# hyeeiin/ECG-Multimodal-Model

Hardware: AMD Instinct MI355X
Metric: samples/sec fwd+bwd, batch-256 multimodal (img+sig+clin), 1->8 MI355X (higher is better)
Workload: dtype bf16; 1 GPU; full multimodal (image 3x224x224 + 5000-pt signal + 16-dim clinical), fwd+bwd+Adam, encoders unfrozen; image_hw=224x224, per_gpu_batch=256, global_batch=256, parallelism=dp1

## Files before the change

ecg-multimodal-model_amd/csrc/elementwise.hip:

```cpp
#include "ops.h"

namespace {

constexpr int EW_THREADS = 256;

__device__ __forceinline__ u32x4 ld16(const void* p) { return *reinterpret_cast<const u32x4*>(p); }
__device__ __forceinline__ u32x4 ld16s(const void* p) {
#ifndef EW_NO_NT
  return __builtin_nontemporal_load(reinterpret_cast<const u32x4*>(p));
#else
  return *reinterpret_cast<const u32x4*>(p);
#endif
}
struct RowDiv { unsigned mul, sh; };
__device__ __forceinline__ long row_div(long r, RowDiv d) { return (long)(((unsigned long long)(unsigned)r * d.mul) >> d.sh); }
static RowDiv make_row_div(int d) {
  unsigned dd = d < 1 ? 1u : (unsigned)d;
  int l = 0;
  while ((1u << l) < dd) ++l;
  RowDiv r;
  r.mul = (unsigned)(((1ull << (31 + l)) + dd - 1) / dd);
  r.sh = 31u + (unsigned)l;
  return r;
}
// ... 362 lines not shown
    }
  }
}

struct BnBwdParams {
  const void* dout;
  const void* maskref;
  const float* gate;
  const float* addc;
  const void* y;
  const float* coef;
  const float* bcoef;
  void* dy;
  void* dz_out;
  float* partial;
  long M;
  int C, rows_per_sample;
  BnBwdFin fin;
  RowDiv rdiv;
  const unsigned char* mask_bits;
};

constexpr int BWD_THREADS = 1024;
template <typename T, bool APPLY>
__global__ __launch_bounds__(BWD_THREADS) void bn_bwd_kernel(BnBwdParams p) {
  constexpr int VEC = Elem<T>::VEC;
  extern __shared__ float shm_dyn[];
  float(*shm)[2 * VEC + 1] = reinterpret_cast<float(*)[2 * VEC + 1]>(shm_dyn);
  const ChanSlice cs = chan_slice(p.C);
  const int cpr = cs.W / VEC, rpi = BWD_THREADS / cpr;
  const int chunk = threadIdx.x % cpr, r0 = threadIdx.x / cpr;
  const int c0 = cs.c_lo + chunk * VEC;
  __shared__ double s_red[APPLY ? FIN_LDS_DOUBLES : 1];
  __shared__ float s_bcoef[APPLY ? 3 * 512 : 1];
  const float* bc = p.bcoef + c0;
  int bcs = p.C;
  const long rfirst = (long)blockIdx.x * rpi + r0;
  u32x4 pd = {}, pv = {};
  bool pre = APPLY && p.fin.partial != nullptr && rfirst < p.M;
  if (pre) {
    pd = ld16s((const T*)p.dout + rfirst * p.C + c0);
    pv = ld16s((const T*)p.y + rfirst * p.C + c0);
  }
  if (APPLY && p.fin.partial) {
    bn_bwd_fin_prologue<BWD_THREADS>(p.fin, p.coef, p.C, cs, s_bcoef, s_red);
    bc = s_bcoef + chunk * VEC;
    bcs = cs.W;
  }
  float mean[VEC], inv[VEC], k1[VEC], k2[VEC], k3[VEC], a1[VEC], a2[VEC], msc[VEC], msh[VEC];
#pragma unroll
  for (int j = 0; j < VEC; ++j) {
    msc[j] = p.coef[c0 + j];
    msh[j] = p.coef[p.C + c0 + j];
    mean[j] = p.coef[2 * p.C + c0 + j];
    inv[j] = p.coef[3 * p.C + c0 + j];
    a1[j] = a2[j] = 0.f;
    if (APPLY) {
      k1[j] = bc[j];
      k2[j] = bc[bcs + j];
      k3[j] = bc[2 * bcs + j];
    }
  }
  const T* dout = (const T*)p.dout;
  const T* mref = (const T*)p.maskref;
  const T* y = (const T*)p.y;
  for (long r = rfirst; r < p.M; r += (long)gridDim.x * rpi) {
    float d[VEC], m[VEC], v[VEC];
    if (pre) {
      unpack16<T>(pd, d);
      unpack16<T>(pv, v);
      pre = false;
    } else {
      unpack16<T>(ld16s(dout + r * p.C + c0), d);
      unpack16<T>(ld16s(y + r * p.C + c0), v);
    }
    if (mref == y) {
#pragma unroll
      for (int j = 0; j < VEC; ++j) d[j] = (v[j] * msc[j] + msh[j]) > 0.f ? d[j] : 0.f;
    } else if (VEC == 8 && p.mask_bits) {
      const unsigned bits = p.mask_bits[r * (p.C / VEC) + c0 / VEC];
#pragma unroll
      for (int j = 0; j < VEC; ++j) d[j] = (bits >> j) & 1u ? d[j] : 0.f;
    } else if (mref) {
      unpack16<T>(ld16s(mref + r * p.C + c0), m);
#pragma unroll
      for (int j = 0; j < VEC; ++j) d[j] = m[j] > 0.f ? d[j] : 0.f;
    }
    if (p.dz_out) st16((T*)p.dz_out + r * p.C + c0, pack16<T>(d));
    if (p.gate) {
      const float* gp = p.gate + row_div(r, p.rdiv) * p.C + c0;
#pragma unroll
      for (int j = 0; j < VEC; ++j) d[j] *= gp[j];
    }
    if (p.addc) {
      const float* ap = p.addc + row_div(r, p.rdiv) * p.C + c0;
#pragma unroll
      for (int j = 0; j < VEC; ++j) d[j] += ap[j];
    }
    if (!APPLY) {
#pragma unroll
      for (int j = 0; j < VEC; ++j) {
        float xh = (v[j] - mean[j]) * inv[j];
        a1[j] += d[j];
        a2[j] += d[j] * xh;
      }
    } else {
      float o[VEC];
#pragma unroll
      for (int j = 0; j < VEC; ++j) {
        float xh = (v[j] - mean[j]) * inv[j];
        o[j] = k1[j] * (d[j] - k2[j] - xh * k3[j]);
      }
      u32x4 pk = pack16<T>(o);
      st16((T*)p.dy + r * p.C + c0, pk);
      if (p.partial) {
        float back[VEC];
        unpack16<T>(pk, back);
#pragma unroll
        for (int j = 0; j < VEC; ++j) a1[j] += back[j];
      }
    }
  }
  if (!APPLY || p.partial) {
    constexpr int NQ = APPLY ? 1 : 2;
#pragma unroll
    for (int j = 0; j < VEC; ++j) {
      shm[threadIdx.x][j] = a1[j];
      if (!APPLY) shm[threadIdx.x][VEC + j] = a2[j];
    }
    __syncthreads();
    for (int o = threadIdx.x; o < NQ * p.C; o += BWD_THREADS) {
      int which = o / p.C, c = o % p.C;
      int ck = c / VEC, j = c % VEC;
      float s = 0.f;
      for (int k = 0; k < rpi; ++k) s += shm[k * cpr + ck][which * VEC + j];
      p.partial[(size_t)blockIdx.x * NQ * p.C + o] = s;
    }
  }
}

__global__ __launch_bounds__(1024) void bn_bwd_finalize_kernel(const float* __restrict__ partial, int rows, int C,
                                                               double count, const float* __restrict__ gamma,
                                                               const float* __restrict__ coef, float* dgamma,
                                                               float* dbeta, float* __restrict__ bcoef, int centered) {
  __shared__ double sh[2][16][64];
  const int c = blockIdx.x * 64 + (threadIdx.x & 63);
  const int slice = threadIdx.x >> 6;
  double s1 = 0.0, s2 = 0.0;
  if (c < C) {
    int r = slice;
    for (; r + 48 < rows; r += 64) {
      float a[4], b[4];
#pragma unroll
      for (int u = 0; u < 4; ++u) {
        const float* row = partial + (size_t)(r + 16 * u) * 2 * C;
        a[u] = row[c];
        b[u] = row[C + c];
      }
#pragma unroll
      for (int u = 0; u < 4; ++u) {
        s1 += (double)a[u];
        s2 += (double)b[u];
      }
    }
    for (; r < rows; r += 16) {
      const float* row = partial + (size_t)r * 2 * C;
      s1 += (double)row[c];
      s2 += (double)row[C + c];
    }
  }
  sh[0][slice][threadIdx.x & 63] = s1;
  sh[1][slice][threadIdx.x & 63] = s2;
  __syncthreads();
  if (slice == 0 && c < C) {
    for (int k = 1; k < 16; ++k) {
      s1 += sh[0][k][threadIdx.x];
      s2 += sh[1][k][threadIdx.x];
    }
    if (centered) s2 *= (double)coef[3 * C + c];
    if (dgamma) dgamma[c] = (float)s2;
    if (dbeta) dbeta[c] = (float)s1;
    bcoef[c] = (gamma ? gamma[c] : 1.f) * coef[3 * C + c];
    bcoef[C + c] = (float)(s1 / count);
    bcoef[2 * C + c] = (float)(s2 / count);
  }
}

__global__ __launch_bounds__(1024) void rows_sum_kernel(const float* __restrict__ partial, int rows, int C, float* out,
                                                        int accumulate) {
  __shared__ double sh[16][64];
  const int c = blockIdx.x * 64 + (threadIdx.x & 63);
  const int slice = threadIdx.x >> 6;
  double s = 0.0;
  if (c < C) {
    int r = slice;
    for (; r + 48 < rows; r += 64) {
      float a[4];
#pragma unroll
      for (int u = 0; u < 4; ++u) a[u] = partial[(size_t)(r + 16 * u) * C + c];
#pragma unroll
      for (int u = 0; u < 4; ++u) s += (double)a[u];
    }
    for (; r < rows; r += 16) s += (double)partial[(size_t)r * C + c];
  }
  sh[slice][threadIdx.x & 63] = s;
  __syncthreads();
  if (slice == 0 && c < C) {
    for (int k = 1; k < 16; ++k) s += sh[k][threadIdx.x];
    out[c] = accumulate ? out[c] + (float)s : (float)s;
  }
}

template <typename T>
__global__ __launch_bounds__(EW_THREADS) void bnrelu_maxpool_kernel(const T* __restrict__ y,
                                                                    const float* __restrict__ coef, T* __restrict__ out,
                                                                    unsigned char* __restrict__ idx, int N, int H,
                                                                    int W, int C, int OH, int OW) {
  constexpr int VEC = Elem<T>::VEC;
  const int cpr = C / VEC;
  long total = (long)N * OH * OW * cpr;
  for (long i = (long)blockIdx.x * blockDim.x + threadIdx.x; i < total; i += (long)gridDim.x * blockDim.x) {
    int chunk = (int)(i % cpr);
    long pix = i / cpr;
    int ow = (int)(pix % OW);
    long t = pix / OW;
    int oh = (int)(t % OH), n = (int)(t / OH);
    int c0 = chunk * VEC;
    float best[VEC];
    int bi[VEC];
    if constexpr (sizeof(T) == 2) {
      unsigned key[VEC];
      float scv[VEC], shv[VEC];
#pragma unroll
      for (int j = 0; j < VEC; ++j) {
        key[j] = 0u;
        scv[j] = coef[c0 + j];
        shv[j] = coef[C + c0 + j];
      }
#pragma unroll
      for (int kh = 0; kh < 3; ++kh) {
        int h = oh * 2 - 1 + kh;
        if ((unsigned)h >= (unsigned)H) continue;
#pragma unroll
        for (int kw = 0; kw < 3; ++kw) {
          int w = ow * 2 - 1 + kw;
          if ((unsigned)w >= (unsigned)W) continue;
          float f[VEC];
          unpack16<T>(ld16(y + (((size_t)n * H + h) * W + w) * C + c0), f);
#pragma unroll
          for (int j = 0; j < VEC; ++j) f[j] = fmaxf(f[j] * scv[j] + shv[j], 0.f);
          const u32x4 r = pack16<bf16_t>(f);
          const unsigned tcode = 15u - (unsigned)(kh * 3 + kw);
#pragma unroll
          for (int q = 0; q < 4; ++q) {
            key[2 * q] = max(key[2 * q], ((r[q] & 0x7fffu) << 4) | tcode);
            key[2 * q + 1] = max(key[2 * q + 1], (((r[q] >> 16) & 0x7fffu) << 4) | tcode);
          }
        }
      }
#pragma unroll
      for (int j = 0; j < VEC; ++j) {
        best[j] = __uint_as_float((key[j] >> 4) << 16);
        bi[j] = 15 - (int)(key[j] & 15u);
      }
    } else {
#pragma unroll
      for (int j = 0; j < VEC; ++j) {
        best[j] = -INFINITY;
        bi[j] = 0;
      }
#pragma unroll
      for (int kh = 0; kh < 3; ++kh) {
        int h = oh * 2 - 1 + kh;
        if ((unsigned)h >= (unsigned)H) continue;
#pragma unroll
        for (int kw = 0; kw < 3; ++kw) {
          int w = ow * 2 - 1 + kw;
          if ((unsigned)w >= (unsigned)W) continue;
          float f[VEC];
          unpack16<T>(ld16(y + (((size_t)n * H + h) * W + w) * C + c0), f);
#pragma unroll
          for (int j = 0; j < VEC; ++j) {
            float a = fmaxf(f[j] * coef[c0 + j] + coef[C + c0 + j], 0.f);
            if (a > best[j]) {
              best[j] = a;
              bi[j] = kh * 3 + kw;
            }
          }
        }
      }
    }
    st16(out + pix * C + c0, pack16<T>(best));
    unsigned pk[VEC / 4];
#pragma unroll
    for (int q = 0; q < VEC / 4; ++q)
      pk[q] = (unsigned)bi[4 * q] | ((unsigned)bi[4 * q + 1] << 8) | ((unsigned)bi[4 * q + 2] << 16) |
              ((unsigned)bi[4 * q + 3] << 24);
    unsigned* ip = reinterpret_cast<unsigned*>(idx + pix * C + c0);
    if constexpr (VEC == 8) *reinterpret_cast<uint2*>(ip) = make_uint2(pk[0], pk[1]);
    else ip[0] = pk[0];
  }
}

template <typename T>
__global__ __launch_bounds__(EW_THREADS) void maxpool_relu_bwd_kernel(const T* __restrict__ dp,
                                                                      const T* __restrict__ pooled,
                                                                      const unsigned char* __restrict__ idx,
                                                                      T* __restrict__ dz, int N, int H, int W, int C,
                                                                      int OH, int OW) {
  constexpr int VEC = Elem<T>::VEC;
  const int cpr = C / VEC;
  const int H2 = (H + 1) >> 1, W2 = (W + 1) >> 1;
  long total = (long)N * H2 * W2 * cpr;
  for (long i = (long)blockIdx.x * blockDim.x + threadIdx.x; i < total; i += (long)gridDim.x * blockDim.x) {
    int chunk = (int)(i % cpr);
    long blk = i / cpr;
    int m = (int)(blk % W2);
    long t = blk / W2;
    int k = (int)(t % H2), n = (int)(t / H2);
    int c0 = chunk * VEC;
    float d[4][VEC], pv[4][VEC];
    unsigned pk[4][2];
    bool wok[4];
#pragma unroll
    for (int a = 0; a < 2; ++a)
#pragma unroll
      for (int b = 0; b < 2; ++b) {
        const int q = a * 2 + b;
        wok[q] = k + a < OH && m + b < OW;
        const size_t o = (((size_t)n * OH + (wok[q] ? k + a : k)) * OW + (wok[q] ? m + b : m)) * C + c0;
        unpack16<T>(ld16(dp + o), d[q]);
        unpack16<T>(ld16(pooled + o), pv[q]);
        if constexpr (VEC == 8) {
          const uint2 t2 = *reinterpret_cast<const uint2*>(idx + o);
          pk[q][0] = t2.x;
          pk[q][1] = t2.y;
        } else {
          pk[q][0] = *reinterpret_cast<const unsigned*>(idx + o);
          pk[q][1] = 0;
        }
      }
    auto g = [&](int q, int tap, int j) -> float {
      const int code = (int)((pk[q][j >> 2] >> (8 * (j & 3))) & 0xffu);
      return (wok[q] && code == tap && pv[q][j] > 0.f) ? d[q][j] : 0.f;
    };
    float o00[VEC], o01[VEC], o10[VEC], o11[VEC];
#pragma unroll
    for (int j = 0; j < VEC; ++j) {
      o00[j] = g(0, 4, j);
      o01[j] = g(0, 5, j) + g(1, 3, j);
      o10[j] = g(0, 7, j) + g(2, 1, j);
      o11[j] = ((g(0, 8, j) + g(1, 6, j)) + g(2, 2, j)) + g(3, 0, j);
    }
    const int h0 = 2 * k, w0 = 2 * m;
    T* base = dz + (((size_t)n * H + h0) * W + w0) * C + c0;
    st16(base, pack16<T>(o00));
    if (w0 + 1 < W) st16(base + C, pack16<T>(o01));
    if (h0 + 1 < H) {
      st16(base + (size_t)W * C, pack16<T>(o10));
      if (w0 + 1 < W) st16(base + (size_t)W * C + C, pack16<T>(o11));
    }
  }
}

template <typename T>
__global__ __launch_bounds__(BWD_THREADS) void pool_bwd_reduce_kernel(const T* __restrict__ dp,
                                                                      const T* __restrict__ pooled,
                                                                      const float* __restrict__ coef,
                                                                      float* __restrict__ partial, long MP, int C) {
  constexpr int VEC = Elem<T>::VEC;
  extern __shared__ float shm_dyn[];
  float(*shm)[2 * VEC + 1] = reinterpret_cast<float(*)[2 * VEC + 1]>(shm_dyn);
  const int cpr = C / VEC, rpi = BWD_THREADS / cpr;
  const int chunk = threadIdx.x % cpr, r0 = threadIdx.x / cpr;
  const int c0 = chunk * VEC;
  float beta[VEC], rsc[VEC], a1[VEC], a2[VEC];
#pragma unroll
  for (int j = 0; j < VEC; ++j) {
    const float sc = coef[c0 + j];
    beta[j] = coef[C + c0 + j] + coef[2 * C + c0 + j] * sc;
    rsc[j] = sc != 0.f ? 1.f / sc : 0.f;
    a1[j] = a2[j] = 0.f;
  }
  for (long r = (long)blockIdx.x * rpi + r0; r < MP; r += (long)gridDim.x * rpi) {
    float d[VEC], v[VEC];
    unpack16<T>(ld16(dp + r * C + c0), d);
    unpack16<T>(ld16(pooled + r * C + c0), v);
#pragma unroll
    for (int j = 0; j < VEC; ++j) {
      const float g = v[j] > 0.f ? d[j] : 0.f;
      a1[j] += g;
      a2[j] += g * (v[j] - beta[j]);
    }
  }
#pragma unroll
  for (int j = 0; j < VEC; ++j) {
    shm[threadIdx.x][j] = a1[j];
    shm[threadIdx.x][VEC + j] = a2[j] * rsc[j];
  }
  __syncthreads();
  for (int o = threadIdx.x; o < 2 * C; o += BWD_THREADS) {
    int which = o / C, c = o % C;
    int ck = c / VEC, j = c % VEC;
    float sum = 0.f;
    for (int k = 0; k < rpi; ++k) sum += shm[k * cpr + ck][which * VEC + j];
    partial[(size_t)blockIdx.x * 2 * C + o] = sum;
  }
}

constexpr int POOL_THREADS = 512;
template <typename T>
__global__ __launch_bounds__(POOL_THREADS) void pool_bn_bwd_apply_kernel(const T* __restrict__ dp,
                                                                         const T* __restrict__ pooled,
                                                                         const unsigned char* __restrict__ idx,
                                                                         const T* __restrict__ y,
                                                                         const float* __restrict__ coef,
                                                                         const float* __restrict__ bcoef,
                                                                         T* __restrict__ dy, float* __restrict__ partial,
                                                                         int N, int H, int W, int C, int OH, int OW) {
  constexpr int VEC = Elem<T>::VEC;
  extern __shared__ float shm_dyn[];
  float(*shm)[VEC + 1] = reinterpret_cast<float(*)[VEC + 1]>(shm_dyn);
  const int cpr = C / VEC;
  const int chunk = threadIdx.x % cpr;
  const int c0 = chunk * VEC;
  const int H2 = (H + 1) >> 1, W2 = (W + 1) >> 1;
  const long nblk = (long)N * H2 * W2;
  const int bpi = POOL_THREADS / cpr;
  float k1[VEC], an[VEC], bn[VEC], a1[VEC];
#pragma unroll
  for (int j = 0; j < VEC; ++j) {
    const float mean = coef[2 * C + c0 + j], inv = coef[3 * C + c0 + j];
    k1[j] = bcoef[c0 + j];
    bn[j] = -k1[j] * bcoef[2 * C + c0 + j] * inv;
    an[j] = -k1[j] * bcoef[C + c0 + j] - bn[j] * mean;
    a1[j] = 0.f;
  }
  for (long blk = (long)blockIdx.x * bpi + threadIdx.x / cpr; blk < nblk; blk += (long)gridDim.x * bpi) {
    int m = (int)(blk % W2);
    long t = blk / W2;
    int k = (int)(t % H2), n = (int)(t / H2);
    const int h0 = 2 * k, w0 = 2 * m;
    const bool okw = w0 + 1 < W, okh = h0 + 1 < H;
    const size_t base = (((size_t)n * H + h0) * W + w0) * C + c0;
    u32x4 rd[4], rp[4], ry[4];
    unsigned pk[4][2];
    bool wok[4];
#pragma unroll
    for (int a = 0; a < 2; ++a)
#pragma unroll
      for (int b = 0; b < 2; ++b) {
        const int q = a * 2 + b;
        wok[q] = k + a < OH && m + b < OW;
        const size_t o = (((size_t)n * OH + (wok[q] ? k + a : k)) * OW + (wok[q] ? m + b : m)) * C + c0;
        rd[q] = ld16(dp + o);
        rp[q] = ld16(pooled + o);
        if constexpr (VEC == 8) {
          const uint2 t2 = *reinterpret_cast<const uint2*>(idx + o);
          pk[q][0] = t2.x;
          pk[q][1] = t2.y;
        } else {
          pk[q][0] = *reinterpret_cast<const unsigned*>(idx + o);
          pk[q][1] = 0;
        }
      }
    ry[0] = ld16(y + base);
    ry[1] = ld16(y + (okw ? base + C : base));
    ry[2] = ld16(y + (okh ? base + (size_t)W * C : base));
    ry[3] = ld16(y + (okh ? base + (size_t)W * C : base) + (okw ? C : 0));
    float d[4][VEC];
#pragma unroll
    for (int q = 0; q < 4; ++q) {
      float pv[VEC];
      unpack16<T>(rd[q], d[q]);
      unpack16<T>(rp[q], pv);
#pragma unroll
      for (int j = 0; j < VEC; ++j) d[q][j] = (wok[q] && pv[j] > 0.f) ? d[q][j] : 0.f;
    }
    auto g = [&](int q, int tap, int j) -> float {
      const int code = (int)((pk[q][j >> 2] >> (8 * (j & 3))) & 0xffu);
      return code == tap ? d[q][j] : 0.f;
    };
    float o[4][VEC];
#pragma unroll
    for (int px = 0; px < 4; ++px) {
      float v[VEC];
      unpack16<T>(ry[px], v);
#pragma unroll
      for (int j = 0; j < VEC; ++j) {
        float z;
        if (px == 0) z = g(0, 4, j);
        else if (px == 1) z = g(0, 5, j) + g(1, 3, j);
        else if (px == 2) z = g(0, 7, j) + g(2, 1, j);
        else z = ((g(0, 8, j) + g(1, 6, j)) + g(2, 2, j)) + g(3, 0, j);
        o[px][j] = k1[j] * z + (bn[j] * v[j] + an[j]);
      }
    }
    const u32x4 p00 = pack16<T>(o[0]), p01 = pack16<T>(o[1]), p10 = pack16<T>(o[2]), p11 = pack16<T>(o[3]);
    st16(dy + base, p00);
    if (okw) st16(dy + base + C, p01);
    if (okh) {
      st16(dy + base + (size_t)W * C, p10);
      if (okw) st16(dy + base + (size_t)W * C + C, p11);
    }
    if (partial) {
      float b0[VEC], b1[VEC], b2[VEC], b3[VEC];
      unpack16<T>(p00, b0); unpack16<T>(p01, b1); unpack16<T>(p10, b2); unpack16<T>(p11, b3);
#pragma unroll
      for (int j = 0; j < VEC; ++j)
        a1[j] += b0[j] + (okw ? b1[j] : 0.f) + (okh ? b2[j] : 0.f) + (okh && okw ? b3[j] : 0.f);
    }
  }
  if (partial) {
#pragma unroll
    for (int j = 0; j < VEC; ++j) shm[threadIdx.x][j] = a1[j];
    __syncthreads();
    for (int c = threadIdx.x; c < C; c += POOL_THREADS) {
      int ck = c / VEC, j = c % VEC;
      float sum = 0.f;
      for (int k = 0; k < bpi; ++k) sum += shm[k * cpr + ck][j];
      partial[(size_t)blockIdx.x * C + c] = sum;
    }
  }
}

template <typename T, bool SEGATE>
__global__ __launch_bounds__(EW_THREADS) void sample_reduce_kernel(const T* __restrict__ x,
                                                                   const T* __restrict__ maskref,
                                                                   const T* __restrict__ y,
                                                                   const float* __restrict__ coef,
                                                                   float* __restrict__ out, int R, int C) {
  constexpr int VEC = Elem<T>::VEC;
  __shared__ float sh[EW_THREADS][VEC + 1];
  const int cpr = C / VEC, nsl = EW_THREADS / cpr;
  const int chunk = threadIdx.x % cpr, slice = threadIdx.x / cpr;
  const int n = blockIdx.x, c0 = chunk * VEC;
  float acc[VEC], sc[VEC], sf[VEC];
#pragma unroll
  for (int j = 0; j < VEC; ++j) {
    acc[j] = 0.f;
    sc[j] = (SEGATE || coef) ? coef[c0 + j] : 1.f;
    sf[j] = (SEGATE || coef) ? coef[C + c0 + j] : 0.f;
  }
  int r = slice;
  if (!SEGATE) {
    for (; r + 3 * nsl < R; r += 4 * nsl) {
      u32x4 q[4];
#pragma unroll
      for (int u = 0; u < 4; ++u) q[u] = ld16(x + ((size_t)n * R + r + u * nsl) * C + c0);
#pragma unroll
      for (int u = 0; u < 4; ++u) {
        float f[VEC];
        unpack16<T>(q[u], f);
#pragma unroll
        for (int j = 0; j < VEC; ++j) acc[j] += f[j];
      }
    }
  }
  for (; r < R; r += nsl) {
    const size_t o = ((size_t)n * R + r) * C + c0;
    float f[VEC];
    unpack16<T>(ld16(x + o), f);
    if (SEGATE) {
      float m[VEC], v[VEC];
      unpack16<T>(ld16(maskref + o), m);
      unpack16<T>(ld16(y + o), v);
#pragma unroll
      for (int j = 0; j < VEC; ++j)
        if (m[j] > 0.f) acc[j] += f[j] * (v[j] * sc[j] + sf[j]);
    } else {
#pragma unroll
      for (int j = 0; j < VEC; ++j) acc[j] += f[j];
    }
  }
#pragma unroll
  for (int j = 0; j < VEC; ++j) sh[threadIdx.x][j] = acc[j];
  __syncthreads();
  for (int c = threadIdx.x; c < C; c += EW_THREADS) {
    const int ck = c / VEC, j = c % VEC;
    float s_ = 0.f;
    for (int k = 0; k < nsl; ++k) s_ += sh[k * cpr + ck][j];
    if (!SEGATE) {
      s_ /= (float)R;
      if (coef) s_ = s_ * coef[c] + coef[C + c];
    }
    out[(size_t)n * C + c] = s_;
  }
}

template <typename T>
__global__ __launch_bounds__(EW_THREADS) void se_gate_bn_kernel(const T* __restrict__ dout, const T* __restrict__ maskref,
                                                                const T* __restrict__ y, const float* __restrict__ coef,
                                                                T* __restrict__ dz, float* __restrict__ dg,
                                                                float* __restrict__ a1o, float* __restrict__ a2o,
                                                                float* __restrict__ a3o, int R, int C) {
  constexpr int VEC = Elem<T>::VEC;
  __shared__ float sh[EW_THREADS][VEC + 1];
  const int cpr = C / VEC, nsl = EW_THREADS / cpr;
  const int chunk = threadIdx.x % cpr, slice = threadIdx.x / cpr;
  const int n = blockIdx.x, c0 = chunk * VEC;
  float sc[VEC], sf[VEC], mu[VEC], ag[VEC], a1[VEC], a2[VEC], a3[VEC];
#pragma unroll
  for (int j = 0; j < VEC; ++j) {
    sc[j] = coef[c0 + j];
    sf[j] = coef[C + c0 + j];
    mu[j] = coef[2 * C + c0 + j];
// ... 203 lines not shown

}

#define DISPATCH_T(dtype, CALL_BF16, CALL_F32, what)                 \
  if ((dtype) == ECGMM_BF16) { CALL_BF16; }                          \
  else if ((dtype) == ECGMM_F32) { CALL_F32; }                       \
  else ECG_FAIL(ECGMM_ERR_DTYPE, what ": bad dtype %d", (int)(dtype))

int ecg_bn_rows(int dtype, long M, int C) {
  int vec = dtype == ECGMM_BF16 ? 8 : 4;
  if (C < vec) return 1;
  int rpi = EW_THREADS / (C / vec);
  int g = ew_grid(M, rpi * 8);
  return g > 1024 ? 1024 : g;
}

static int fold_rows(const float*& partial, int& rows, int width, hipStream_t stream) {
  if (rows <= 512) return 0;
  float* tail = const_cast<float*>(partial) + (size_t)rows * width;
  int chunk = ceil_div(rows, ECG_TAIL_ROWS);
  int nb = ceil_div(rows, chunk);
  hipLaunchKernelGGL(rows_stage1_kernel, dim3(ceil_div(width, 64), nb), dim3(1024), 0, stream, partial, rows, width,
                     chunk, tail);
  ECG_CHECK_LAUNCH("rows_stage1");
  partial = tail;
  rows = nb;
  return 0;
}

int ecg_bn_finalize(const float* partial, int rows, int C, double count, const float* gamma, const float* beta,
                    float* rm, float* rv, long long* nbt, float momentum, float eps, float* coef,
                    hipStream_t stream) {
  ECG_TRY(fold_rows(partial, rows, 2 * C, stream));
  hipLaunchKernelGGL(bn_finalize_kernel, dim3(ceil_div(C, 64)), dim3(1024), 0, stream, partial, rows, C, count, gamma,
                     beta, rm, rv, nbt, momentum, eps, coef);
  ECG_CHECK_LAUNCH("bn_finalize");
  return 0;
}

int ecg_bn_eval_coef(int C, const float* gamma, const float* beta, const float* rm, const float* rv, float eps,
                     float* coef, hipStream_t stream) {
  hipLaunchKernelGGL(bn_eval_coef_kernel, dim3(ceil_div(C, 256)), dim3(256), 0, stream, C, gamma, beta, rm, rv, eps,
                     coef);
  ECG_CHECK_LAUNCH("bn_eval_coef");
  return 0;
}

int ecg_col_stats(int dtype, const void* x, long M, int C, float* partial, int* rows_out, hipStream_t stream) {
  if (!chunk_ok(C, dtype)) ECG_FAIL(ECGMM_ERR_SHAPE, "col_stats: C=%d unsupported", C);
  int grid = ecg_bn_rows(dtype, M, C);
  *rows_out = grid;
  DISPATCH_T(dtype,
             hipLaunchKernelGGL(col_stats_kernel<bf16_t>, dim3(grid), dim3(EW_THREADS), 0, stream, (const bf16_t*)x, M,
                                C, partial),
             hipLaunchKernelGGL(col_stats_kernel<float>, dim3(grid), dim3(EW_THREADS), 0, stream, (const float*)x, M, C,
                                partial),
             "col_stats");
  ECG_CHECK_LAUNCH("col_stats");
  return 0;
}

bool ecg_bn_fold_ok(int C, int rows) {
  if (!sw::BN_FOLD.get() || rows < 1 || rows > 512 || C > 512) return false;
  return C >= 128 ? C % 128 == 0 : (C >= 16 && 1024 % C == 0);
}

static int bn_fold_slices(int C) {
  return sw::BN_FOLD_SLICE.get() && C >= 256 && C % 128 == 0 ? C / 128 : 1;
}
static dim3 bn_fold_grid(int dtype, long M, int C, int ns, int threads, int trips) {
  const int vec = dtype == ECGMM_BF16 ? 8 : 4;
  int gx = ew_grid(M, (threads / (C / ns / vec)) * trips);
  if (gx > 256 / ns) gx = 256 / ns;
  return dim3(gx, ns);
}

int ecg_bn_act_fold(int dtype, const void* y, float* coef, const EcgBnFold& f, const void* res, const float* rcoef,
                    const float* gate, int rows_per_sample, int relu, void* out, long M, int C, hipStream_t stream,
                    unsigned char* relu_bits) {
  if (!chunk_ok(C, dtype)) ECG_FAIL(ECGMM_ERR_SHAPE, "bn_act: C=%d unsupported", C);
  if (!ecg_bn_fold_ok(C, f.rows)) ECG_FAIL(ECGMM_ERR_SHAPE, "bn_act_fold: C=%d rows=%d not foldable", C, f.rows);
  BnActParams p;
  memset(&p, 0, sizeof(p));
  p.y = y; p.coef = coef; p.res = res; p.rcoef = rcoef; p.gate = gate; p.out = out; p.M = M; p.C = C;
  p.rows_per_sample = rows_per_sample > 0 ? rows_per_sample : 1; p.relu = relu;
  p.rdiv = make_row_div(p.rows_per_sample);
  p.fin.partial = f.partial; p.fin.rows = f.rows; p.fin.count = f.count; p.fin.gamma = f.gamma; p.fin.beta = f.beta;
  p.fin.rm = f.rm; p.fin.rv = f.rv; p.fin.nbt = f.nbt; p.fin.momentum = f.momentum; p.fin.eps = f.eps; p.fin.coef_out = coef;
  p.relu_bits = dtype == ECGMM_BF16 && relu ? relu_bits : nullptr;
  const dim3 grid = bn_fold_grid(dtype, M, C, bn_fold_slices(C), BN_ACT_THREADS, 4);
  DISPATCH_T(dtype, hipLaunchKernelGGL(bn_act_kernel<bf16_t>, grid, dim3(BN_ACT_THREADS), 0, stream, p),
             hipLaunchKernelGGL(bn_act_kernel<float>, grid, dim3(BN_ACT_THREADS), 0, stream, p), "bn_act");
  ECG_CHECK_LAUNCH("bn_act_fold");
  return 0;
}

int ecg_bn_act(int dtype, const void* y, const float* coef, const void* res, const float* rcoef, const float* gate,
               int rows_per_sample, int relu, void* out, long M, int C, hipStream_t stream, unsigned char* relu_bits) {
  if (!chunk_ok(C, dtype)) ECG_FAIL(ECGMM_ERR_SHAPE, "bn_act: C=%d unsupported", C);
  BnActParams p;
  memset(&p, 0, sizeof(p));
  p.y = y; p.coef = coef; p.res = res; p.rcoef = rcoef; p.gate = gate; p.out = out; p.M = M; p.C = C;
  p.rows_per_sample = rows_per_sample > 0 ? rows_per_sample : 1; p.relu = relu;
  p.rdiv = make_row_div(p.rows_per_sample);
  p.relu_bits = dtype == ECGMM_BF16 && relu ? relu_bits : nullptr;
  int vec = dtype == ECGMM_BF16 ? 8 : 4;
  int grid = ew_grid(M, (BN_ACT_THREADS / (C / vec)) * 4);
  if (grid > 256) grid = 256;
  DISPATCH_T(dtype, hipLaunchKernelGGL(bn_act_kernel<bf16_t>, dim3(grid), dim3(BN_ACT_THREADS), 0, stream, p),
             hipLaunchKernelGGL(bn_act_kernel<float>, dim3(grid), dim3(BN_ACT_THREADS), 0, stream, p), "bn_act");
  ECG_CHECK_LAUNCH("bn_act");
  return 0;
}

static int bn_bwd_rows(int dtype, long M, int C) {
  int vec = dtype == ECGMM_BF16 ? 8 : 4;
  if (C < vec) return 1;
  int rpi = BWD_THREADS / (C / vec);
  int g = ew_grid(M, rpi * 8);
  return g > 256 ? 256 : g;
}
template <typename T, bool APPLY>
static void bn_bwd_launch(const BnBwdParams& p, dim3 grid, hipStream_t stream) {
  constexpr size_t lds = (size_t)BWD_THREADS * (2 * Elem<T>::VEC + 1) * sizeof(float);
  static bool attr_set = false;
  if (!attr_set) {
    (void)hipFuncSetAttribute((const void*)bn_bwd_kernel<T, APPLY>, hipFuncAttributeMaxDynamicSharedMemorySize, (int)lds);
    attr_set = true;
  }
  hipLaunchKernelGGL((bn_bwd_kernel<T, APPLY>), grid, dim3(BWD_THREADS), lds, stream, p);
}
static dim3 bn_bwd_apply_grid(int dtype, const BnBwdParams& p, int rows) {
  if (!p.fin.partial || p.partial) return dim3(rows);
  return bn_fold_grid(dtype, p.M, p.C, bn_fold_slices(p.C), BWD_THREADS, 8);
}

size_t ecg_bn_bwd_scratch(int dtype, long M, int C) {
  return ((size_t)(bn_bwd_rows(dtype, M, C) + ECG_TAIL_ROWS) * 2 * C + 3 * C) * sizeof(float);
}

int ecg_bn_bwd(int dtype, const void* dout, const void* maskref, const float* gate, const float* addc,
               int rows_per_sample, const void* y, const float* coef, const float* gamma, float* dgamma, float* dbeta,
               void* dy, void* dz_out, float* dbias, long M, int C, float* scratch, hipStream_t stream,
               const unsigned char* mask_bits) {
  if (!chunk_ok(C, dtype)) ECG_FAIL(ECGMM_ERR_SHAPE, "bn_bwd: C=%d unsupported", C);
  if (dtype != ECGMM_BF16 || maskref == y) mask_bits = nullptr;
  int grid = bn_bwd_rows(dtype, M, C);
  float* partial = scratch;
  float* bcoef = scratch + (size_t)(grid + ECG_TAIL_ROWS) * 2 * C;
  BnBwdParams p;
  memset(&p, 0, sizeof(p));
  p.dout = dout; p.maskref = maskref; p.gate = gate; p.addc = addc; p.y = y; p.coef = coef; p.M = M; p.C = C;
  p.rows_per_sample = rows_per_sample > 0 ? rows_per_sample : 1;
  p.rdiv = make_row_div(p.rows_per_sample);
  p.partial = partial;
  p.mask_bits = mask_bits;
  const bool dz_early = dy && dz_out && (mask_bits || (maskref && maskref != y)) && dz_out != dout;
  if (dz_early) p.dz_out = dz_out;
  DISPATCH_T(dtype, (bn_bwd_launch<bf16_t, false>(p, grid, stream)), (bn_bwd_launch<float, false>(p, grid, stream)), "bn_bwd");
  ECG_CHECK_LAUNCH("bn_bwd_reduce");
  const bool fold = dy && !dbias && ecg_bn_fold_ok(C, grid);
  if (!fold) {
    const float* pr = partial;
    int rows = grid;
    hipLaunchKernelGGL(bn_bwd_finalize_kernel, dim3(ceil_div(C, 64)), dim3(1024), 0, stream, pr, rows, C, (double)M,
                       gamma, coef, dgamma, dbeta, bcoef, 0);
    ECG_CHECK_LAUNCH("bn_bwd_finalize");
  }
  if (!dy) return 0;
  p.bcoef = bcoef; p.dy = dy; p.dz_out = dz_out;
  if (fold) {
    p.fin.partial = partial; p.fin.rows = grid; p.fin.count = (double)M; p.fin.gamma = gamma; p.fin.dgamma = dgamma;
    p.fin.dbeta = dbeta; p.fin.centered = 0;
  }
  if (dz_early) { p.dout = dz_out; p.maskref = nullptr; p.mask_bits = nullptr; p.dz_out = nullptr; }
  p.partial = dbias ? partial : nullptr;
  const dim3 agrid = bn_bwd_apply_grid(dtype, p, grid);
  DISPATCH_T(dtype, (bn_bwd_launch<bf16_t, true>(p, agrid, stream)), (bn_bwd_launch<float, true>(p, agrid, stream)), "bn_bwd");
  ECG_CHECK_LAUNCH("bn_bwd_apply");
  if (dbias) {
    hipLaunchKernelGGL(rows_sum_kernel, dim3(ceil_div(C, 64)), dim3(1024), 0, stream, partial, grid, C, dbias, 0);
    ECG_CHECK_LAUNCH("rows_sum");
  }
  return 0;
}

int ecg_bn_bwd_tail(int dtype, const void* dout, const void* maskref, const void* y, const float* coef,
                    const float* gamma, float* dgamma, float* dbeta, void* dy, const float* partial, int rows, long M,
                    int C, float* scratch, hipStream_t stream, const float* gate, const float* addc,
                    int rows_per_sample, float* dbias) {
  if (!chunk_ok(C, dtype)) ECG_FAIL(ECGMM_ERR_SHAPE, "bn_bwd: C=%d unsupported", C);
  if (rows < 1 || rows > 512) ECG_FAIL(ECGMM_ERR_SHAPE, "bn_bwd_tail: %d partial rows (1..512)", rows);
  const int grid = bn_bwd_rows(dtype, M, C);
  float* bcoef = scratch + (size_t)(grid + ECG_TAIL_ROWS) * 2 * C;
  const bool fold = ecg_bn_fold_ok(C, rows);
  if (!fold) {
    hipLaunchKernelGGL(bn_bwd_finalize_kernel, dim3(ceil_div(C, 64)), dim3(1024), 0, stream, partial, rows, C, (double)M,
                       gamma, coef, dgamma, dbeta, bcoef, 1);
    ECG_CHECK_LAUNCH("bn_bwd_finalize");
  }
  BnBwdParams p;
  memset(&p, 0, sizeof(p));
  p.dout = dout; p.maskref = maskref; p.y = y; p.coef = coef; p.M = M; p.C = C;
  p.gate = gate; p.addc = addc; p.rows_per_sample = rows_per_sample > 0 ? rows_per_sample : 1;
  p.rdiv = make_row_div(p.rows_per_sample);
  p.bcoef = bcoef; p.dy = dy;
  if (fold) {
    p.fin.partial = partial; p.fin.rows = rows; p.fin.count = (double)M; p.fin.gamma = gamma; p.fin.dgamma = dgamma;
    p.fin.dbeta = dbeta; p.fin.centered = 1;
  }
  p.partial = dbias ? scratch : nullptr;
  const dim3 agrid = bn_bwd_apply_grid(dtype, p, grid);
  DISPATCH_T(dtype, (bn_bwd_launch<bf16_t, true>(p, agrid, stream)), (bn_bwd_launch<float, true>(p, agrid, stream)), "bn_bwd");
  ECG_CHECK_LAUNCH("bn_bwd_apply");
  if (dbias) {
    hipLaunchKernelGGL(rows_sum_kernel, dim3(ceil_div(C, 64)), dim3(1024), 0, stream, (const float*)scratch, grid, C, dbias, 0);
    ECG_CHECK_LAUNCH("rows_sum");
  }
  return 0;
}

template <typename T>
static void pool_bwd_launch(const void* dp, const void* pooled, const unsigned char* idx, const void* y, const float* coef,
                            const float* gamma, float* dgamma, float* dbeta, void* dy, float* dbias, int N, int H, int W,
                            int C, int OH, int OW, float* scratch, int rows, hipStream_t stream) {
  constexpr int VEC = Elem<T>::VEC;
  constexpr size_t lds2 = (size_t)BWD_THREADS * (2 * VEC + 1) * sizeof(float), ldsp = (size_t)POOL_THREADS * (VEC + 1) * sizeof(float);
  static bool attr_set = false;
  if (!attr_set) {
    (void)hipFuncSetAttribute((const void*)pool_bwd_reduce_kernel<T>, hipFuncAttributeMaxDynamicSharedMemorySize, (int)lds2);
    attr_set = true;
  }
  const long MP = (long)N * OH * OW, M = (long)N * H * W;
  float* partial = scratch;
  float* bcoef = scratch + (size_t)(rows + ECG_TAIL_ROWS) * 2 * C;
  const int rpi = BWD_THREADS / (C / VEC);
  int g1 = ew_grid(MP, rpi * 8);
  g1 = g1 > rows ? rows : g1;
  hipLaunchKernelGGL(pool_bwd_reduce_kernel<T>, dim3(g1), dim3(BWD_THREADS), lds2, stream, (const T*)dp, (const T*)pooled,
                     coef, partial, MP, C);
  hipLaunchKernelGGL(bn_bwd_finalize_kernel, dim3(ceil_div(C, 64)), dim3(1024), 0, stream, (const float*)partial, g1, C,
                     (double)M, gamma, coef, dgamma, dbeta, bcoef, 1);
  const long nblk = (long)N * ((H + 1) / 2) * ((W + 1) / 2);
  int g2 = ew_grid(nblk, POOL_THREADS / (C / VEC));
  if (dbias && g2 > rows) g2 = rows;
  hipLaunchKernelGGL(pool_bn_bwd_apply_kernel<T>, dim3(g2), dim3(POOL_THREADS), dbias ? ldsp : 0, stream, (const T*)dp,
                     (const T*)pooled, idx, (const T*)y, coef, (const float*)bcoef, (T*)dy, dbias ? partial : nullptr, N, H, W,
                     C, OH, OW);
  if (dbias) hipLaunchKernelGGL(rows_sum_kernel, dim3(ceil_div(C, 64)), dim3(1024), 0, stream, (const float*)partial, g2, C, dbias, 0);
}

int ecg_pool_bn_bwd_reduce(int dtype, const void* dp, const void* pooled, const float* coef, const float* gamma, float* dgamma,
                           float* dbeta, int N, int H, int W, int C, float* scratch, const float** bcoef_out,
                           hipStream_t stream) {
  if (dtype != ECGMM_BF16) ECG_FAIL(ECGMM_ERR_DTYPE, "pool_bn_bwd_reduce: bf16 only");
  if (!chunk_ok(C, dtype)) ECG_FAIL(ECGMM_ERR_SHAPE, "pool_bn_bwd_reduce: C=%d unsupported", C);
  using T = bf16_t;
  constexpr int VEC = Elem<T>::VEC;
  constexpr size_t lds2 = (size_t)BWD_THREADS * (2 * VEC + 1) * sizeof(float);
  static bool attr_set = false;
  if (!attr_set) {
    (void)hipFuncSetAttribute((const void*)pool_bwd_reduce_kernel<T>, hipFuncAttributeMaxDynamicSharedMemorySize, (int)lds2);
    attr_set = true;
  }
  const int OH = (H - 1) / 2 + 1, OW = (W - 1) / 2 + 1;
  const int rows = bn_bwd_rows(dtype, (long)N * H * W, C);
  const long MP = (long)N * OH * OW, M = (long)N * H * W;
  float* partial = scratch;
  float* bcoef = scratch + (size_t)(rows + ECG_TAIL_ROWS) * 2 * C;
  const int rpi = BWD_THREADS / (C / VEC);
  int g1 = ew_grid(MP, rpi * 8);
  g1 = g1 > rows ? rows : g1;
  hipLaunchKernelGGL(pool_bwd_reduce_kernel<T>, dim3(g1), dim3(BWD_THREADS), lds2, stream, (const T*)dp, (const T*)pooled, coef,
                     partial, MP, C);
  ECG_CHECK_LAUNCH("pool_bwd_reduce");
  hipLaunchKernelGGL(bn_bwd_finalize_kernel, dim3(ceil_div(C, 64)), dim3(1024), 0, stream, (const float*)partial, g1, C,
                     (double)M, gamma, coef, dgamma, dbeta, bcoef, 1);
  ECG_CHECK_LAUNCH("bn_bwd_finalize");
  *bcoef_out = bcoef;
  return 0;
}

bool ecg_stem_fuse_on() { return sw::STEM_FUSE.get() != 0; }

int ecg_pool_bn_bwd(int dtype, const void* dp, const void* pooled, const unsigned char* idx, const void* y,
                    const float* coef, const float* gamma, float* dgamma, float* dbeta, void* dy, float* dbias, int N,
                    int H, int W, int C, float* scratch, hipStream_t stream) {
  if (!chunk_ok(C, dtype)) ECG_FAIL(ECGMM_ERR_SHAPE, "pool_bn_bwd: C=%d unsupported", C);
  const int OH = (H - 1) / 2 + 1, OW = (W - 1) / 2 + 1;
  const int rows = bn_bwd_rows(dtype, (long)N * H * W, C);
  DISPATCH_T(dtype, (pool_bwd_launch<bf16_t>(dp, pooled, idx, y, coef, gamma, dgamma, dbeta, dy, dbias, N, H, W, C, OH, OW, scratch, rows, stream)),
             (pool_bwd_launch<float>(dp, pooled, idx, y, coef, gamma, dgamma, dbeta, dy, dbias, N, H, W, C, OH, OW, scratch, rows, stream)),
             "pool_bn_bwd");
  ECG_CHECK_LAUNCH("pool_bn_bwd");
  return 0;
}

int ecg_rows_sum(const float* partial, int rows, int C, float* out, int accumulate, hipStream_t stream) {
  hipLaunchKernelGGL(rows_sum_kernel, dim3(ceil_div(C, 64)), dim3(1024), 0, stream, partial, rows, C, out, accumulate);
  ECG_CHECK_LAUNCH("rows_sum");
  return 0;
}

int ecg_bnrelu_maxpool(int dtype, const void* y, const float* coef, void* out, unsigned char* idx, int N, int H, int W,
                       int C, hipStream_t stream) {
  if (!chunk_ok(C, dtype)) ECG_FAIL(ECGMM_ERR_SHAPE, "maxpool: C=%d unsupported", C);
  int OH = (H + 2 - 3) / 2 + 1, OW = (W + 2 - 3) / 2 + 1;
  int vec = dtype == ECGMM_BF16 ? 8 : 4;
  int grid = ew_grid((long)N * OH * OW * (C / vec), EW_THREADS);
  DISPATCH_T(dtype,
             hipLaunchKernelGGL(bnrelu_maxpool_kernel<bf16_t>, dim3(grid), dim3(EW_THREADS), 0, stream,
                                (const bf16_t*)y, coef, (bf16_t*)out, idx, N, H, W, C, OH, OW),
             hipLaunchKernelGGL(bnrelu_maxpool_kernel<float>, dim3(grid), dim3(EW_THREADS), 0, stream, (const float*)y,
                                coef, (float*)out, idx, N, H, W, C, OH, OW),
             "maxpool");
  ECG_CHECK_LAUNCH("bnrelu_maxpool");
  return 0;
}

int ecg_maxpool_relu_bwd(int dtype, const void* dp, const void* pooled, const unsigned char* idx, void* dz, int N,
                         int H, int W, int C, hipStream_t stream) {
  if (!chunk_ok(C, dtype)) ECG_FAIL(ECGMM_ERR_SHAPE, "maxpool bwd: C=%d unsupported", C);
  int OH = (H + 2 - 3) / 2 + 1, OW = (W + 2 - 3) / 2 + 1;
  int vec = dtype == ECGMM_BF16 ? 8 : 4;
  int grid = ew_grid((long)N * ((H + 1) / 2) * ((W + 1) / 2) * (C / vec), EW_THREADS);
  DISPATCH_T(dtype,
             hipLaunchKernelGGL(maxpool_relu_bwd_kernel<bf16_t>, dim3(grid), dim3(EW_THREADS), 0, stream,
                                (const bf16_t*)dp, (const bf16_t*)pooled, idx, (bf16_t*)dz, N, H, W, C, OH, OW),
             hipLaunchKernelGGL(maxpool_relu_bwd_kernel<float>, dim3(grid), dim3(EW_THREADS), 0, stream,
                                (const float*)dp, (const float*)pooled, idx, (float*)dz, N, H, W, C, OH, OW),
             "maxpool bwd");
  ECG_CHECK_LAUNCH("maxpool_relu_bwd");
  return 0;
}

int ecg_avgpool(int dtype, const void* x, float* out, int N, int R, int C, const float* coef, hipStream_t stream) {
  if (!chunk_ok(C, dtype)) ECG_FAIL(ECGMM_ERR_SHAPE, "avgpool: C=%d unsupported", C);
  DISPATCH_T(dtype,
             hipLaunchKernelGGL((sample_reduce_kernel<bf16_t, false>), dim3(N), dim3(EW_THREADS), 0, stream,
                                (const bf16_t*)x, (const bf16_t*)nullptr, (const bf16_t*)nullptr, coef, out, R, C),
             hipLaunchKernelGGL((sample_reduce_kernel<float, false>), dim3(N), dim3(EW_THREADS), 0, stream,
                                (const float*)x, (const float*)nullptr, (const float*)nullptr, coef, out, R, C),
             "avgpool");
  ECG_CHECK_LAUNCH("avgpool");
  return 0;
}

int ecg_bcast_rows(int dtype, const float* v, void* out, int N, int R, int C, float scale, hipStream_t stream) {
  long total = (long)N * R * C;
  const int vecw = dtype == ECGMM_BF16 ? 8 : 4;
  if (C % vecw == 0 && C / vecw <= 1024 && 1024 % (C / vecw) == 0 && ((uintptr_t)out & 15) == 0) {
    const long M = (long)N * R;
    int g = ew_grid(M, (1024 / (C / vecw)) * 4);
    if (g > 256) g = 256;
    DISPATCH_T(dtype,
               hipLaunchKernelGGL(bcast_rows_vec_kernel<bf16_t>, dim3(g), dim3(1024), 0, stream, v, (bf16_t*)out, M, make_row_div(R), C, scale),
               hipLaunchKernelGGL(bcast_rows_vec_kernel<float>, dim3(g), dim3(1024), 0, stream, v, (float*)out, M, make_row_div(R), C, scale),
               "bcast_rows");
    ECG_CHECK_LAUNCH("bcast_rows_vec");
    return 0;
  }
  int grid = ew_grid(total, 256);
  DISPATCH_T(dtype,
             hipLaunchKernelGGL(bcast_rows_kernel<bf16_t>, dim3(grid), dim3(256), 0, stream, v, (bf16_t*)out, total, R,
                                C, scale),
             hipLaunchKernelGGL(bcast_rows_kernel<float>, dim3(grid), dim3(256), 0, stream, v, (float*)out, total, R, C,
                                scale),
             "bcast_rows");
  ECG_CHECK_LAUNCH("bcast_rows");
  return 0;
}

int ecg_se_gate_grad(int dtype, const void* dout, const void* maskref, const void* y, const float* coef, float* dg,
                     int N, int R, int C, hipStream_t stream) {
  if (!chunk_ok(C, dtype)) ECG_FAIL(ECGMM_ERR_SHAPE, "se_gate_grad: C=%d unsupported", C);
  DISPATCH_T(dtype,
             hipLaunchKernelGGL((sample_reduce_kernel<bf16_t, true>), dim3(N), dim3(EW_THREADS), 0, stream,
                                (const bf16_t*)dout, (const bf16_t*)maskref, (const bf16_t*)y, coef, dg, R, C),
             hipLaunchKernelGGL((sample_reduce_kernel<float, true>), dim3(N), dim3(EW_THREADS), 0, stream,
                                (const float*)dout, (const float*)maskref, (const float*)y, coef, dg, R, C),
             "se_gate_grad");
  ECG_CHECK_LAUNCH("se_gate_grad");
  return 0;
}

int ecg_se_gate_bn(int dtype, const void* dout, const void* maskref, const void* y, const float* coef, void* dz,
                   float* dg, float* a1, float* a2, float* a3, int N, int R, int C, hipStream_t stream) {
  if (!chunk_ok(C, dtype)) ECG_FAIL(ECGMM_ERR_SHAPE, "se_gate_bn: C=%d unsupported", C);
  DISPATCH_T(dtype,
             hipLaunchKernelGGL(se_gate_bn_kernel<bf16_t>, dim3(N), dim3(EW_THREADS), 0, stream, (const bf16_t*)dout,
                                (const bf16_t*)maskref, (const bf16_t*)y, coef, (bf16_t*)dz, dg, a1, a2, a3, R, C),
             hipLaunchKernelGGL(se_gate_bn_kernel<float>, dim3(N), dim3(EW_THREADS), 0, stream, (const float*)dout,
                                (const float*)maskref, (const float*)y, coef, (float*)dz, dg, a1, a2, a3, R, C),
             "se_gate_bn");
  ECG_CHECK_LAUNCH("se_gate_bn");
  return 0;
}
int ecg_se_bn_rows(const float* a1, const float* a2, const float* a3, const float* gate, const float* addc, int N, int R,
                   int C, float* rows, hipStream_t stream) {
  hipLaunchKernelGGL(se_bn_rows_kernel, dim3(ceil_div(C, 64), SE_ROWS), dim3(256), 0, stream, a1, a2, a3, gate, addc, N, R,
                     C, rows);
  ECG_CHECK_LAUNCH("se_bn_rows");
  return 0;
}
int ecg_se_bn_nrows() { return SE_ROWS; }

int ecg_pack_weight(int dtype, const float* w_oihw, void* fwd, void* dgrad, int Cout, int Cin, int RS,
                    hipStream_t stream) {
  long total = (long)Cout * Cin * RS;
  int grid = ew_grid(total, 256);
  DISPATCH_T(dtype,
             hipLaunchKernelGGL(pack_weight_kernel<bf16_t>, dim3(grid), dim3(256), 0, stream, w_oihw, (bf16_t*)fwd,
                                (bf16_t*)dgrad, Cout, Cin, RS),
             hipLaunchKernelGGL(pack_weight_kernel<float>, dim3(grid), dim3(256), 0, stream, w_oihw, (float*)fwd,
                                (float*)dgrad, Cout, Cin, RS),
             "pack_weight");
  ECG_CHECK_LAUNCH("pack_weight");
  return 0;
}

int ecg_pack_weight_batch(int dtype, const EcgPackItem* items, int n, hipStream_t stream) {
  for (int base = 0; base < n; base += ECG_PACK_MAX) {
    PackBatch b;
    memset(&b, 0, sizeof(b));
    b.n = n - base < ECG_PACK_MAX ? n - base : ECG_PACK_MAX;
    int blocks = 0;
    for (int i = 0; i < b.n; ++i) {
      const EcgPackItem& it = items[base + i];
      b.w[i] = it.w; b.fwd[i] = it.fwd; b.dgr[i] = it.dgrad; b.cout[i] = it.Cout; b.cin[i] = it.Cin; b.rs[i] = it.RS;
      b.blk0[i] = blocks;
      if (it.RS > 9) ECG_FAIL(ECGMM_ERR_SHAPE, "pack_weight_batch: %d taps unsupported (<= 9)", it.RS);
      blocks += ceil_div(it.Cout, 32) * ceil_div(it.Cin, 32);
    }
    b.blk0[b.n] = blocks;
    DISPATCH_T(dtype, hipLaunchKernelGGL(pack_weight_batch_kernel<bf16_t>, dim3(blocks), dim3(256), 0, stream, b),
               hipLaunchKernelGGL(pack_weight_batch_kernel<float>, dim3(blocks), dim3(256), 0, stream, b), "pack_weight_batch");
    ECG_CHECK_LAUNCH("pack_weight_batch");
  }
  return 0;
}

int ecg_nchw_to_nhwc(int dtype, const float* src, void* dst, int N, int C, long HW, hipStream_t stream) {
  dim3 grid(ceil_div(HW, 32), ceil_div(C, 32), N);
  DISPATCH_T(dtype,
             hipLaunchKernelGGL((nchw_nhwc_kernel<bf16_t, true>), grid, dim3(256), 0, stream, src, dst, C, HW),
             hipLaunchKernelGGL((nchw_nhwc_kernel<float, true>), grid, dim3(256), 0, stream, src, dst, C, HW),
             "nchw_to_nhwc");
  ECG_CHECK_LAUNCH("nchw_to_nhwc");
  return 0;
}

int ecg_nhwc_to_nchw(int dtype, const void* src, float* dst, int N, int C, long HW, hipStream_t stream) {
  dim3 grid(ceil_div(HW, 32), ceil_div(C, 32), N);
  DISPATCH_T(dtype,
             hipLaunchKernelGGL((nchw_nhwc_kernel<bf16_t, false>), grid, dim3(256), 0, stream, src, dst, C, HW),
             hipLaunchKernelGGL((nchw_nhwc_kernel<float, false>), grid, dim3(256), 0, stream, src, dst, C, HW),
             "nhwc_to_nchw");
  ECG_CHECK_LAUNCH("nhwc_to_nchw");
  return 0;
}

int ecg_cast(int dtype, const float* src, void* dst, long n, hipStream_t stream) {
  int grid = ew_grid(n, 256);
  DISPATCH_T(dtype, hipLaunchKernelGGL(cast_kernel<bf16_t>, dim3(grid), dim3(256), 0, stream, src, (bf16_t*)dst, n),
             hipLaunchKernelGGL(cast_kernel<float>, dim3(grid), dim3(256), 0, stream, src, (float*)dst, n), "cast");
  ECG_CHECK_LAUNCH("cast");
  return 0;
}
int ecg_uncast(int dtype, const void* src, float* dst, long n, hipStream_t stream) {
  int grid = ew_grid(n, 256);
  DISPATCH_T(dtype,
             hipLaunchKernelGGL(uncast_kernel<bf16_t>, dim3(grid), dim3(256), 0, stream, (const bf16_t*)src, dst, n),
             hipLaunchKernelGGL(uncast_kernel<float>, dim3(grid), dim3(256), 0, stream, (const float*)src, dst, n),
             "uncast");
  ECG_CHECK_LAUNCH("uncast");
  return 0;
}
```

Before: 39850 samples/s.

## Add LDS-tiled BN+ReLU+maxpool kernel for bf16 C=64 stems

Adds a tiled kernel for the fused BN-affine+ReLU+3x3/s2 maxpool when dtype is bf16 and C=64. Each block stages a halo band of the input into shared memory (normalised and ReLU'd once per element, swizzled to avoid bank conflicts) and computes an 8x8 (or 1x64 for 1-D signals) output tile from it. This avoids the roughly 2.25x redundant global reads and repeated BN math of the per-output gather kernel. The argmax is taken with a packed integer key (magnitude bits plus tap code), which relies on post-ReLU values being non-negative. It adds a __syncthreads and LDS use per block.

Measured after the change: 40110 samples/s (median of 6 runs). About the same (+0.7%).

```diff
diff --git a/ecg-multimodal-model_amd/csrc/elementwise.hip b/ecg-multimodal-model_amd/csrc/elementwise.hip
--- a/ecg-multimodal-model_amd/csrc/elementwise.hip
+++ b/ecg-multimodal-model_amd/csrc/elementwise.hip
@@ -688,6 +688,98 @@
   }
 }
 
+constexpr int PT_THREADS = 256;
+template <int TOH, int TOW, bool ONE_D>
+__global__ __launch_bounds__(PT_THREADS) void bnrelu_maxpool_tile_kernel(const bf16_t* __restrict__ y,
+                                                                         const float* __restrict__ coef,
+                                                                         bf16_t* __restrict__ out,
+                                                                         unsigned char* __restrict__ idx, int H, int W,
+                                                                         int OH, int OW) {
+  constexpr int C = 64, VEC = 8;
+  constexpr int BR = ONE_D ? 1 : 2 * TOH + 1;
+  constexpr int MC = 2 * TOW, BW = MC + 2;
+  constexpr int PPT = PT_THREADS / 8;
+  constexpr int TRIPS = (BR * MC + PPT - 1) / PPT;
+  static_assert((MC & (MC - 1)) == 0 && (TOW & (TOW - 1)) == 0 && (TOH * TOW) % PPT == 0 && BR * 8 <= PT_THREADS, "tile shape");
+  __shared__ u32x4 band[BR * BW * 8];
+  const int tid = threadIdx.x, k = tid & 7, pos = tid >> 3, c0 = k * VEC;
+  const int ow0 = blockIdx.x * TOW, oh0 = blockIdx.y * TOH;
+  const int hb = ONE_D ? 0 : 2 * oh0 - 1, wb = 2 * ow0 - 1;
+  const bf16_t* yn = y + (size_t)blockIdx.z * H * W * C + c0;
+  float scv[VEC], shv[VEC];
+#pragma unroll
+  for (int j = 0; j < VEC; ++j) {
+    scv[j] = coef[c0 + j];
+    shv[j] = coef[C + c0 + j];
+  }
+  auto put = [&](const u32x4& raw, int br, int bw) {
+    float f[VEC];
+    unpack16<bf16_t>(raw, f);
+#pragma unroll
+    for (int j = 0; j < VEC; ++j) f[j] = fmaxf(f[j] * scv[j] + shv[j], 0.f);
+    band[(br * BW + (bw ^ ((bw >> 1) & 1))) * 8 + k] = pack16<bf16_t>(f);
+  };
+  auto at = [&](int h, int w) {
+    const int hc = min(max(h, 0), H - 1), wc = min(max(w, 0), W - 1);
+    return ld16(yn + (unsigned)(hc * W + wc) * C);
+  };
+  u32x4 v[TRIPS], ve;
+#pragma unroll
+  for (int t = 0; t < TRIPS; ++t) {
+    const int q = pos + PPT * t;
+    v[t] = at(hb + q / MC, wb + (q & (MC - 1)));
+  }
+  const bool extra = tid < BR * 8;
+  if (extra) ve = at(hb + pos, wb + MC);
+#pragma unroll
+  for (int t = 0; t < TRIPS; ++t) {
+    const int q = pos + PPT * t, br = q / MC, bw = q & (MC - 1);
+    if (br < BR && (unsigned)(hb + br) < (unsigned)H && (unsigned)(wb + bw) < (unsigned)W) put(v[t], br, bw);
+  }
+  if (extra && (unsigned)(hb + pos) < (unsigned)H && (unsigned)(wb + MC) < (unsigned)W) put(ve, pos, MC);
+  __syncthreads();
+  bf16_t* on = out + (size_t)blockIdx.z * OH * OW * C + c0;
+  unsigned char* in = idx + (size_t)blockIdx.z * OH * OW * C + c0;
+#pragma unroll
+  for (int it = 0; it < TOH * TOW / PPT; ++it) {
+    const int p = pos + PPT * it, r = p / TOW, c = p & (TOW - 1);
+    const int oh = oh0 + r, ow = ow0 + c;
+    if (oh >= OH || ow >= OW) continue;
+    unsigned key[VEC];
+#pragma unroll
+    for (int j = 0; j < VEC; ++j) key[j] = 0u;
+#pragma unroll
+    for (int kh = 0; kh < 3; ++kh) {
+      const int h = oh * 2 - 1 + kh;
+      if ((unsigned)h >= (unsigned)H) continue;
+#pragma unroll
+      for (int kw = 0; kw < 3; ++kw) {
+        const int w = ow * 2 - 1 + kw;
+        if ((unsigned)w >= (unsigned)W) continue;
+        const int bw = 2 * c + kw;
+        const u32x4 r4 = band[((h - hb) * BW + (bw ^ ((bw >> 1) & 1))) * 8 + k];
+        const unsigned tcode = 15u - (unsigned)(kh * 3 + kw);
+#pragma unroll
+        for (int q = 0; q < 4; ++q) {
+          key[2 * q] = max(key[2 * q], ((r4[q] & 0x7fffu) << 4) | tcode);
+          key[2 * q + 1] = max(key[2 * q + 1], (((r4[q] >> 16) & 0x7fffu) << 4) | tcode);
+        }
+      }
+    }
+    float best[VEC];
+    unsigned bi[VEC];
+#pragma unroll
+    for (int j = 0; j < VEC; ++j) {
+      best[j] = __uint_as_float((key[j] >> 4) << 16);
+      bi[j] = 15u - (key[j] & 15u);
+    }
+    const unsigned o = (unsigned)(oh * OW + ow) * C;
+    st16(on + o, pack16<bf16_t>(best));
+    *reinterpret_cast<uint2*>(in + o) = make_uint2(bi[0] | (bi[1] << 8) | (bi[2] << 16) | (bi[3] << 24),
+                                                   bi[4] | (bi[5] << 8) | (bi[6] << 16) | (bi[7] << 24));
+  }
+}
+
 template <typename T>
 __global__ __launch_bounds__(EW_THREADS) void maxpool_relu_bwd_kernel(const T* __restrict__ dp,
                                                                       const T* __restrict__ pooled,
@@ -1497,10 +1589,28 @@
   return 0;
 }
 
+static bool pool_tile_ok(int N, int H, int W, int C) {
+#ifdef EW_NO_POOL_TILE
+  return false;
+#else
+  return C == 64 && N >= 1 && N <= 65535 && H >= 1 && W >= 1 && (long)H * W * C < (1L << 31) && H <= 65535 * 8;
+#endif
+}
+
 int ecg_bnrelu_maxpool(int dtype, const void* y, const float* coef, void* out, unsigned char* idx, int N, int H, int W,
                        int C, hipStream_t stream) {
   if (!chunk_ok(C, dtype)) ECG_FAIL(ECGMM_ERR_SHAPE, "maxpool: C=%d unsupported", C);
   int OH = (H + 2 - 3) / 2 + 1, OW = (W + 2 - 3) / 2 + 1;
+  if (dtype == ECGMM_BF16 && pool_tile_ok(N, H, W, C)) {
+    if (H == 1)
+      hipLaunchKernelGGL((bnrelu_maxpool_tile_kernel<1, 64, true>), dim3(ceil_div(OW, 64), 1, N), dim3(PT_THREADS), 0, stream,
+                         (const bf16_t*)y, coef, (bf16_t*)out, idx, H, W, OH, OW);
+    else
+      hipLaunchKernelGGL((bnrelu_maxpool_tile_kernel<8, 8, false>), dim3(ceil_div(OW, 8), ceil_div(OH, 8), N), dim3(PT_THREADS),
+                         0, stream, (const bf16_t*)y, coef, (bf16_t*)out, idx, H, W, OH, OW);
+    ECG_CHECK_LAUNCH("bnrelu_maxpool_tile");
+    return 0;
+  }
   int vec = dtype == ECGMM_BF16 ? 8 : 4;
   int grid = ew_grid((long)N * OH * OW * (C / vec), EW_THREADS);
   DISPATCH_T(dtype,
```
